# TritonDataCenter/registrar

Hardware: AMD Instinct MI355X
Metric: ephemeral registrations/sec (higher is better)
Workload: dtype n/a; 1 GPU; model=registrar re-register cycle, 1k ephemeral znodes/proc, global_batch=1000, parallelism=1 registrar procs (1/GPU), shared synthetic ZK ensemble (1 server) on rank 0, znodes_per_proc=1000, step=cleanup(1k unlink) + mkdirp + 1k ephemeral create + 1k-node heartbeat

## Files before the change

registrar_amd/csrc/bindings.cpp:

```cpp
#include <pybind11/pybind11.h>
#include <pybind11/stl.h>

#include "ensemble.hpp"
#include "gpu.hpp"
#include "health.hpp"
#include "json.hpp"
#include "log.hpp"
#include "orchestrator.hpp"
#include "registrar.hpp"
#include "zkclient.hpp"

namespace py = pybind11;
using namespace registrar;

namespace {

LogLevel level_from(const std::string& name) {
  LogLevel l = LogLevel::Warn;
  log_level_from_name(name, &l);
  return l;
}

Logger make_logger(const std::string& name, const std::string& level) {
  Logger log(name);
  log.set_level(level_from(level));
  return log;
}

py::dict stat_to_dict(const zk::Stat& st) {
  py::dict d;
  d["czxid"] = st.czxid;
  d["mzxid"] = st.mzxid;
  d["ctime"] = st.ctime;
  d["mtime"] = st.mtime;
  d["version"] = st.version;
  d["cversion"] = st.cversion;
  d["ephemeralOwner"] = st.ephemeral_owner;
  d["dataLength"] = st.data_length;
  d["numChildren"] = st.num_children;
  d["pzxid"] = st.pzxid;
  return d;
}

py::dict session_event_to_dict(const zk::SessionEvent& ev) {
  py::dict d;
  d["type"] = zk::session_event_name(ev.type);
  d["session_id"] = ev.session_id;
  d["attempt"] = ev.attempt;
  d["delay_ms"] = ev.delay_ms;
  return d;
}

py::dict orch_event_to_dict(const OrchEvent& ev) {
  py::dict d;
  d["type"] = orch_event_name(ev.type);
  d["detail"] = ev.detail;
  d["znodes"] = ev.znodes;
  d["rtt_us"] = ev.rtt_us;
  return d;
}
// ... 280 lines not shown
               rc = c.multi(mops, &per_op);
             }
             return py::make_tuple(rc, per_op);
           },
           py::arg("ops"))
      .def("heartbeat",
           [](zk::ZkClient& c, const std::vector<std::string>& nodes, const py::dict& retry) {
             zk::RetryPolicy rp = retry_from_dict(retry);
             int64_t rtt = 0;
             int rc;
             {
               py::gil_scoped_release rel;
               rc = c.heartbeat(nodes, rp, &rtt);
             }
             return py::make_tuple(rc, rtt);
           },
           py::arg("nodes"), py::arg("retry") = py::dict());

  m.def("domain_to_path", &domain_to_path);
  m.def("self_hostname", &self_hostname);
  m.def("self_address", &self_address, py::arg("admin_ip") = "");
  m.def("build_host_record",
        [](const std::string& registration_json) {
          return build_host_record(parse_registration(Json::parse(registration_json))).dump();
        });
  m.def("build_service_record",
        [](const std::string& registration_json) {
          return build_service_record(parse_registration(Json::parse(registration_json))).dump();
        });
  m.def("build_node_list",
        [](const std::string& registration_json) {
          return build_node_list(parse_registration(Json::parse(registration_json)));
        });
  py::class_<PreparedRegistration>(m, "PreparedRegistration")
      .def(py::init([](const std::string& registration_json) {
             return std::make_unique<PreparedRegistration>(
                 prepare_registration(parse_registration(Json::parse(registration_json))));
           }),
           py::arg("registration_json"))
      .def_property_readonly("path", [](const PreparedRegistration& p) { return p.path; })
      .def_property_readonly("nodes", [](const PreparedRegistration& p) { return p.nodes; })
      .def_property_readonly("host_payload",
                             [](const PreparedRegistration& p) { return py::bytes(p.host_payload); })
      .def("register_",
           [](PreparedRegistration& prep, zk::ZkClient& c, const std::string& log_level) {
             Logger log = make_logger("registrar", log_level);
             RegisterResult res;
             {
               py::gil_scoped_release rel;
               res = register_prepared(c, prep, log);
             }
             return py::make_tuple(res.rc, res.error, res.znodes());
           },
           py::arg("client"), py::arg("log_level") = "warn")
      .def("heartbeat",
           [](PreparedRegistration& prep, zk::ZkClient& c, const py::dict& retry) {
             zk::RetryPolicy rp = retry_from_dict(retry);
             int64_t rtt = 0;
             int rc;
             {
               py::gil_scoped_release rel;
               rc = heartbeat_prepared(c, prep, rp, &rtt);
             }
             return py::make_tuple(rc, rtt);
           },
           py::arg("client"), py::arg("retry") = py::dict());

  m.def("register_node",
        [](zk::ZkClient& c, const std::string& registration_json, const std::string& log_level) {
          RegistrationConfig cfg = parse_registration(Json::parse(registration_json));
          Logger log = make_logger("registrar", log_level);
          RegisterResult res;
          {
            py::gil_scoped_release rel;
            res = register_node(c, cfg, log);
          }
          return py::make_tuple(res.rc, res.error, res.znodes());
        },
        py::arg("client"), py::arg("registration_json"), py::arg("log_level") = "warn");
  m.def("unregister_node",
        [](zk::ZkClient& c, const std::vector<std::string>& znodes, const std::string& log_level) {
          Logger log = make_logger("registrar", log_level);
          py::gil_scoped_release rel;
          return unregister_node(c, znodes, log);
        },
        py::arg("client"), py::arg("znodes"), py::arg("log_level") = "warn");

  m.def("exec_with_timeout",
        [](const std::string& command, int64_t timeout_ms) {
          ExecResult res;
          {
            py::gil_scoped_release rel;
            res = exec_with_timeout(command, timeout_ms);
          }
          py::dict d;
// ... 100 lines not shown
```

registrar_amd/csrc/ensemble.cpp:

```cpp
#include "ensemble.hpp"

#include "node_store.hpp"

#include <arpa/inet.h>
#include <fcntl.h>
#include <netinet/in.h>
#include <netinet/tcp.h>
#include <sys/socket.h>
#include <unistd.h>

#include <algorithm>
#include <array>
#include <cstdio>
#include <future>

namespace registrar {
namespace zk {

using namespace detail;

namespace {

void set_nonblock(int fd) {
  int fl = fcntl(fd, F_GETFL, 0);
  fcntl(fd, F_SETFL, fl | O_NONBLOCK);
}

void set_nodelay(int fd) {
  int one = 1;
  setsockopt(fd, IPPROTO_TCP, TCP_NODELAY, &one, sizeof(one));
}

inline void spin_pause() {
#if defined(__x86_64__) || defined(__i386__)
  __builtin_ia32_pause();
// ... 409 lines not shown
        maybe_elect_leader_locked();
      }
      set_nodelay(fd);
      auto conn = std::make_shared<Conn>();
      conn->id = next_conn_id.fetch_add(1);
      conn->fd = fd;
      conn->server_idx = server_idx;
      conn->io_idx = next_io.fetch_add(1) % loops.size();
      uint64_t cid = conn->id;
      size_t io_idx = conn->io_idx;
      {
        std::lock_guard<std::mutex> g(conns_mu);
        conns[cid] = conn;
      }
      loops[io_idx]->add_fd(fd, EPOLLIN, [this, cid](uint32_t ev) { on_conn_event(cid, ev); });
    }
  }

  ConnPtr lookup(uint64_t cid) {
    std::lock_guard<std::mutex> g(conns_mu);
    auto it = conns.find(cid);
    return it == conns.end() ? nullptr : it->second;
  }

  void on_conn_event(uint64_t cid, uint32_t ev) {
    ConnPtr c = lookup(cid);
    if (!c) return;
    if (c->dead.load() || (ev & (EPOLLHUP | EPOLLERR))) {
      close_conn(c.get());
      return;
    }
    if (ev & EPOLLIN) {
      bool eof = false;
      while (true) {
        size_t room = 0;
        char* dst = c->inbuf.tail(65536, &room);
        ssize_t n = read(c->fd, dst, room);
        if (n > 0) {
          c->inbuf.commit(static_cast<size_t>(n));
        } else if (n == 0) {
          eof = true;
          break;
        } else {
          if (errno == EAGAIN || errno == EWOULDBLOCK) break;
          if (errno == EINTR) continue;
          eof = true;
          break;
        }
      }
      c->drain_mono_ms = now_ms();
      c->drain_wall_ms = wall_ms();
      c->last_parent = PathRef{std::string_view(), 0};
      {
        std::lock_guard<std::mutex> og(c->out_mu);
        c->draining = true;
      }
      if (!process_frames(c.get())) return;
      flush_out(c.get(), true);
      if (c->dead.load()) return;
      if (eof) {
        close_conn(c.get());
        return;
      }
      return;
    }
    if (ev & EPOLLOUT) flush_out(c.get());
  }

  bool process_frames(Conn* c) {
    struct CarryScope {
      Conn* c;
      Carry carry;
      explicit CarryScope(Conn* cc) : c(cc) { c->carry = &carry; }
      ~CarryScope() {
        carry.release();
        c->carry = nullptr;
      }
    } scope(c);
    while (!c->dead.load()) {
      size_t avail = c->inbuf.size();
      if (avail < 4) break;
      const unsigned char* p = reinterpret_cast<const unsigned char*>(c->inbuf.ptr());
      uint32_t len = (static_cast<uint32_t>(p[0]) << 24) | (static_cast<uint32_t>(p[1]) << 16) |
                     (static_cast<uint32_t>(p[2]) << 8) | static_cast<uint32_t>(p[3]);
      if (len > 4 * 1024 * 1024) {
        close_conn(c);
        return false;
      }
      if (avail < 4 + len) break;
      const char* body = c->inbuf.ptr() + 4;
      c->inbuf.consume(4 + len);
// ... 1440 lines not shown
```

registrar_amd/csrc/hotpath_main.cpp:

```cpp
#include <dirent.h>
#include <signal.h>
#include <sys/syscall.h>
#include <unistd.h>

#include <atomic>
#include <chrono>
#include <cstdio>
#include <cstdlib>
#include <cstring>
#include <new>
#include <set>
#include <string>
#include <vector>

#include "ensemble.hpp"
#include "registrar.hpp"
#include "zkclient.hpp"

#ifdef HOTPATH_PROF
#if !defined(__x86_64__)
#error "hotpath-prof reads x86-64 registers from the signal context"
#endif
#include <cxxabi.h>
#include <dlfcn.h>
#include <sys/time.h>
#include <ucontext.h>

#include <algorithm>
#include <map>
#endif

using namespace registrar;


namespace {
struct AllocSlot {
  std::atomic<long> tid{0};
  std::atomic<uint64_t> count{0};
  std::atomic<uint64_t> bytes{0};
};
constexpr int kMaxSlots = 256;
AllocSlot g_slots[kMaxSlots];
std::atomic<int> g_next_slot{0};
thread_local AllocSlot* t_slot = nullptr;

inline void count_alloc(size_t n) {
  AllocSlot* s = t_slot;
  if (!s) {
    int i = g_next_slot.fetch_add(1);
    if (i >= kMaxSlots) return;
// ... 222 lines not shown
  }
  return buf;
}

void prof_report() {
  size_t n = g_nsamples;
  fprintf(stderr,
          "\nhotpath-prof: %zu samples on ens-io, %zu ticks on other threads (ITIMER_PROF asked for 1 ms; the kernel "
          "delivers at its own tick rate)\n",
          n, static_cast<size_t>(g_other_thread));
  if (!n) return;
  std::map<std::string, size_t> self, chains;
  for (size_t i = 0; i < n; i++) {
    const ProfSample& s = g_samples[i];
    self[symbol_of(s.pc[0], false)]++;
    std::string c = symbol_of(s.pc[0], false);
    for (int d = 1; d < 4; d++) c += " <- " + symbol_of(s.pc[d], true);
    chains[c]++;
  }
  auto top = [&](const std::map<std::string, size_t>& m, size_t k, const char* title) {
    std::vector<std::pair<size_t, std::string>> v;
    for (auto& kv : m) v.push_back({kv.second, kv.first});
    std::sort(v.begin(), v.end(), [](auto& a, auto& b) { return a.first > b.first; });
    fprintf(stderr, "--- %s ---\n", title);
    for (size_t i = 0; i < v.size() && i < k; i++)
      fprintf(stderr, "%6.2f%% %6zu  %s\n", 100.0 * v[i].first / n, v[i].first, v[i].second.c_str());
  };
  top(self, 40, "self time per symbol");
  top(chains, 25, "most common 4-deep chains (leaf <- callers)");
}
}
#endif

int main(int argc, char** argv) {
  signal(SIGPIPE, SIG_IGN);
  int n = argc > 1 ? atoi(argv[1]) : 1000;
  int steps = argc > 2 ? atoi(argv[2]) : 200;
  int warmup = argc > 3 ? atoi(argv[3]) : 20;
  if (n < 1 || steps < 1 || warmup < 0) {
    fprintf(stderr, "usage: hotpath [N znodes >= 1] [K steps >= 1] [warmup >= 0]\n");
    return 2;
  }

  Logger log("hotpath");
  log.set_level(LogLevel::Warn);
  long caller_tid = syscall(SYS_gettid);
  name_thread(caller_tid, "caller");

  zk::EnsembleConfig ecfg;
  ecfg.ports = {0};
  ecfg.io_threads = 1;
  ecfg.max_session_timeout_ms = 60000;
  zk::Ensemble ens(ecfg);
  std::set<long> before = list_tids();
  ens.start();
  std::vector<long> ens_tids = new_tids(before);
  if (ens_tids.size() != 1) {
    fprintf(stderr, "hotpath: expected 1 ensemble IO thread, found %zu\n", ens_tids.size());
    return 1;
  }
  long ens_tid = ens_tids[0];
  name_thread(ens_tid, "ens-io");

  zk::ZkClientConfig ccfg;
  ccfg.servers.push_back({"127.0.0.1", ens.ports()[0]});
  ccfg.session_timeout_ms = 40000;
// ... 15 lines not shown
  reg.admin_ip = "127.0.0.1";
  reg.hostname = "bench-r0";
  reg.settle_ms = 0;
  for (int i = 0; i < n - 1; i++) {
    char buf[64];
    snprintf(buf, sizeof(buf), "a%04d.rank0.bench.mi355x", i);
    reg.aliases.push_back(buf);
  }
  PreparedRegistration prep = prepare_registration(reg);
  zk::RetryPolicy retry;

  auto step = [&](Sample* ens_mid) -> bool {
    RegisterResult res = register_prepared(client, prep, log);
    if (res.rc != zk::kZOk) {
      fprintf(stderr, "hotpath: register failed: %s\n", res.error.c_str());
      return false;
    }
    if (ens_mid) *ens_mid = sample_allocs(ens_tid);
    int64_t rtt = 0;
    int rc = heartbeat_prepared(client, prep, retry, &rtt);
    if (rc != zk::kZOk) {
      fprintf(stderr, "hotpath: heartbeat failed: %s\n", zk::error_name(rc));
      return false;
    }
    return true;
  };

  for (int i = 0; i < warmup; i++)
    if (!step(nullptr)) return 1;

#ifdef HOTPATH_PROF
  if (!prof_arm(ens_tid)) return 1;
#endif

  const long tids[3] = {ens_tid, cli_tid, caller_tid};
  const char* names[3] = {"ens-io", "zk-loop", "caller"};
  Sample s0[3], s1[3];
  uint64_t ens_reg_allocs = 0, ens_hb_allocs = 0;
  auto c0 = ens.counters();
  for (int t = 0; t < 3; t++) s0[t] = sample(tids[t]);
  double t0 = now_s();
  for (int i = 0; i < steps; i++) {
    Sample a = sample_allocs(ens_tid), mid;
    if (!step(&mid)) return 1;
    Sample b = sample_allocs(ens_tid);
    ens_reg_allocs += mid.allocs - a.allocs;
    ens_hb_allocs += b.allocs - mid.allocs;
  }
  double wall = now_s() - t0;
  for (int t = 0; t < 3; t++) s1[t] = sample(tids[t]);
  auto c1 = ens.counters();
  double locks_step = static_cast<double>(c1["tree_locks"] - c0["tree_locks"]) / steps;
  double locks_register = locks_step - static_cast<double>(c1["exists"] - c0["exists"]) / steps;
#ifdef HOTPATH_PROF
  prof_disarm();
#endif

  int del_rounds = steps < 5 ? steps : 5;
  uint64_t ens_del_allocs = 0;
  for (int i = 0; i < del_rounds; i++) {
    Sample a = sample_allocs(ens_tid);
    std::vector<int> rcs = client.delete_many(prep.nodes);
    Sample b = sample_allocs(ens_tid);
    for (int rc : rcs)
      if (rc != zk::kZOk) {
        fprintf(stderr, "hotpath: delete failed: %s\n", zk::error_name(rc));
        return 1;
      }
    ens_del_allocs += b.allocs - a.allocs;
    if (!step(nullptr)) return 1;
  }

  auto counters = ens.counters();
  client.close();
  ens.stop();

  double k = static_cast<double>(steps);
  fprintf(stderr, "hotpath: N=%d znodes, %d steps (+%d warmup), wall %.3f ms/step\n", n, steps, warmup,
          wall / k * 1e3);
  fprintf(stderr, "%-8s %12s %14s %14s\n", "thread", "cpu_us/step", "allocs/step", "bytes/step");
  for (int t = 0; t < 3; t++)
    fprintf(stderr, "%-8s %12.1f %14.1f %14.0f\n", names[t], (s1[t].cpu - s0[t].cpu) / k / 1e3,
            (s1[t].allocs - s0[t].allocs) / k, (s1[t].bytes - s0[t].bytes) / k);
  fprintf(stderr, "ens-io allocs by phase: register %.1f/step, heartbeat(exists) %.1f/step, delete-only %.1f/batch\n",
          ens_reg_allocs / k, ens_hb_allocs / k, ens_del_allocs / static_cast<double>(del_rounds));
  fprintf(stderr, "tree locks: %.1f/step, of which register %.1f/step\n", locks_step, locks_register);

  printf("{\"tool\": \"hotpath\", \"znodes\": %d, \"steps\": %d, \"warmup\": %d, \"wall_ms_per_step\": %.4f", n,
         steps, warmup, wall / k * 1e3);
  const char* keys[3] = {"ens_io", "zk_loop", "caller"};
  for (int t = 0; t < 3; t++)
    printf(", \"%s\": {\"cpu_us_per_step\": %.1f, \"allocs_per_step\": %.1f, \"bytes_per_step\": %.0f}", keys[t],
           (s1[t].cpu - s0[t].cpu) / k / 1e3, (s1[t].allocs - s0[t].allocs) / k, (s1[t].bytes - s0[t].bytes) / k);
  printf(", \"ens_io_allocs_register_per_step\": %.1f, \"ens_io_allocs_heartbeat_per_step\": %.1f"
         ", \"ens_io_allocs_delete_per_batch\": %.1f",
         ens_reg_allocs / k, ens_hb_allocs / k, ens_del_allocs / static_cast<double>(del_rounds));
  printf(", \"tree_locks_per_step\": %.1f, \"tree_locks_register_per_step\": %.1f", locks_step, locks_register);
  printf(", \"requests\": {\"create\": %llu, \"delete\": %llu, \"exists\": %llu}}\n",
         static_cast<unsigned long long>(counters["create"]), static_cast<unsigned long long>(counters["delete"]),
         static_cast<unsigned long long>(counters["exists"]));
#ifdef HOTPATH_PROF
  prof_report();
#endif
  return 0;
}
```

registrar_amd/csrc/stress_main.cpp:

```cpp
#include <dirent.h>
#include <execinfo.h>
#include <signal.h>
#include <sys/syscall.h>
#include <unistd.h>

#include <atomic>
#include <chrono>
#include <cstdio>
#include <cstring>
#include <thread>
#include <vector>

#include "ensemble.hpp"
#include "node_store.hpp"
#include "registrar.hpp"
#include "zkclient.hpp"

using namespace registrar;

namespace {
void dump_backtrace(int) {
  void* frames[48];
  int n = backtrace(frames, 48);
  char hdr[64];
  int len = snprintf(hdr, sizeof(hdr), "--- thread %ld backtrace ---\n", syscall(SYS_gettid));
  ssize_t r = write(2, hdr, len);
  (void)r;
  backtrace_symbols_fd(frames, n, 2);
}

void arm_watchdog(int seconds) {
  struct sigaction sa;
  memset(&sa, 0, sizeof(sa));
  sa.sa_handler = dump_backtrace;
  sigaction(SIGUSR1, &sa, nullptr);
  std::thread([seconds] {
    std::this_thread::sleep_for(std::chrono::seconds(seconds));
    fprintf(stderr, "WATCHDOG: run overshot %ds; dumping all threads\n", seconds);
    DIR* d = opendir("/proc/self/task");
    if (d) {
      while (struct dirent* e = readdir(d)) {
        if (e->d_name[0] == '.') continue;
        long tid = atol(e->d_name);
        syscall(SYS_tgkill, getpid(), tid, SIGUSR1);
        std::this_thread::sleep_for(std::chrono::milliseconds(150));
      }
      closedir(d);
    }
    std::this_thread::sleep_for(std::chrono::seconds(1));
    _exit(42);
  }).detach();
}
bool crossed_phase(int seconds, const Logger& log) {
  zk::EnsembleConfig ecfg;
  ecfg.ports = {0};
  ecfg.io_threads = 2;
  ecfg.tick_ms = 50;
  ecfg.log_level = LogLevel::Error;
  zk::Ensemble ens(ecfg);
  ens.start();
  int port = ens.ports()[0];
  auto make_client = [&] {
    zk::ZkClientConfig ccfg;
    ccfg.servers.push_back({"127.0.0.1", port});
    ccfg.session_timeout_ms = 30000;
    ccfg.log_level = LogLevel::Fatal;
    auto c = std::make_unique<zk::ZkClient>(std::move(ccfg), log);
    c->start();
    return c;
  };
  std::unique_ptr<zk::ZkClient> cl[2] = {make_client(), nullptr};
  if (!cl[0]->wait_connected(5000)) return false;
  cl[1] = make_client();
  if (!cl[1]->wait_connected(5000)) return false;
  auto reader = make_client();
  if (!reader->wait_connected(5000)) return false;
  const std::string parent[2] = {"/x/p0", "/x/p1"};
  if (cl[0]->mkdirp(parent[0]) != zk::kZOk || cl[0]->mkdirp(parent[1]) != zk::kZOk) return false;

  constexpr int kBatch = 96;
  auto batch_of = [&](int who) {
    std::vector<std::string> paths;
    for (int j = 0; j < kBatch; j++) {
      int under = ((j / 8) % 2 == 0) ? who : 1 - who;
      paths.push_back(parent[under] + "/s" + std::to_string(who) + "_" + std::to_string(j));
// ... 225 lines not shown
          break;
        }
        case 2: {
          for (size_t i = 0; i < 3; i++)
            if (!ens.server_up(i)) ens.restart_server(i);
          break;
        }
        default:
          ens.set_latency_ms(static_cast<int>(next() % 3));
          break;
      }
    }
    ens.set_latency_ms(0);
    for (size_t i = 0; i < 3; i++)
      if (!ens.server_up(i)) ens.restart_server(i);
  };

  for (int phase = 0; phase < 2; phase++) {
    bool contested = phase == 1;
    int secs = contested ? contested_seconds : seconds;
    if (secs <= 0) continue;
    stop.store(false);
    std::vector<std::thread> threads;
    for (int i = 0; i < nclients; i++) threads.emplace_back(client_fn, i, contested);
    std::thread chaos(chaos_fn);
    std::this_thread::sleep_for(std::chrono::seconds(secs));
    stop.store(true);
    for (auto& t : threads) t.join();
    chaos.join();
  }

  bool crossed_ok = crossed_secs <= 0 || crossed_phase(crossed_secs, log);
  bool treelock_ok = treelock_phase();

  auto deadline = std::chrono::steady_clock::now() + std::chrono::seconds(15);
  while (!ens.session_ids().empty() && std::chrono::steady_clock::now() < deadline)
    std::this_thread::sleep_for(std::chrono::milliseconds(20));
  size_t sessions_left = ens.session_ids().size();
  std::vector<std::string> violations = ens.audit();
  deadline = std::chrono::steady_clock::now() + std::chrono::seconds(2);
  while (!violations.empty() && std::chrono::steady_clock::now() < deadline) {
    std::this_thread::sleep_for(std::chrono::milliseconds(20));
    violations = ens.audit();
  }
  size_t ephemerals_left = ens.ephemeral_count();
  ens.stop();

  printf("stress: %llu cycles, %llu hard failures, %llu contested cycles\n",
         static_cast<unsigned long long>(cycles.load()), static_cast<unsigned long long>(failures.load()),
         static_cast<unsigned long long>(contested_cycles.load()));
  bool sound = true;
  if (sessions_left != 0) {
    printf("stress: %zu sessions still alive after every client closed\n", sessions_left);
    sound = false;
  }
  if (ephemerals_left != 0) {
    printf("stress: %zu ephemerals left\n", ephemerals_left);
    sound = false;
  }
  for (const auto& v : violations) {
    printf("stress: audit: %s\n", v.c_str());
    sound = false;
  }
  if (contested_seconds > 0 && contested_cycles.load() == 0) {
    printf("stress: the contested phase completed no cycle\n");
    sound = false;
  }
  bool behaved = cycles.load() > 0 && failures.load() < cycles.load() / 4 + 16;
  if (!crossed_ok) printf("stress: the crossed-parents phase failed\n");
  if (!treelock_ok) printf("stress: the tree lock phase failed\n");
  return (behaved && sound && crossed_ok && treelock_ok) ? 0 : 1;
}
```

registrar_amd/csrc/zkclient.cpp:

```cpp
#include "zkclient.hpp"

#include <arpa/inet.h>
#include <fcntl.h>
#include <netdb.h>
#include <netinet/in.h>
#include <netinet/tcp.h>
#include <sys/socket.h>
#include <unistd.h>

#include <algorithm>
#include <chrono>
#include <future>
#include <thread>
#include <unordered_set>

namespace registrar {
namespace zk {

const char* session_event_name(SessionEvent::Type t) {
  switch (t) {
    case SessionEvent::Type::Connected:
      return "connect";
    case SessionEvent::Type::Disconnected:
      return "close";
    case SessionEvent::Type::Expired:
      return "session_expired";
    case SessionEvent::Type::ConnectAttempt:
      return "attempt";
    case SessionEvent::Type::Closed:
      return "closed";
  }
  return "?";
}
// ... 269 lines not shown
  void teardown_socket() {
    if (conn_timer) {
      loop.cancel(conn_timer);
      conn_timer = 0;
    }
    if (ping_timer) {
      loop.cancel(ping_timer);
      ping_timer = 0;
    }
    if (fd >= 0) {
      loop.del_fd(fd);
      ::close(fd);
      fd = -1;
    }
    inbuf.clear();
    outbuf.clear();
    flush_scheduled = false;
  }

  void fail_all_pending(int rc) {
    std::deque<Pending> q;
    q.swap(pending);
    for (auto& p : q) {
      if (p.rcs)
        fail_batch(p, rc);
      else if (p.done)
        p.done(rc, nullptr);
    }
  }


  bool read_frames() {
    bool eof = false;
    while (true) {
      size_t room = 0;
      char* dst = inbuf.tail(65536, &room);
      ssize_t n = read(fd, dst, room);
      if (n > 0) {
        inbuf.commit(static_cast<size_t>(n));
      } else if (n == 0) {
        eof = true;
        break;
      } else {
        if (errno == EAGAIN || errno == EWOULDBLOCK) break;
        if (errno == EINTR) continue;
        eof = true;
        break;
      }
    }
    last_recv = now_ms();
    while (true) {
      size_t avail = inbuf.size();
      if (avail < 4) break;
      const unsigned char* p = reinterpret_cast<const unsigned char*>(inbuf.ptr());
      uint32_t len = (static_cast<uint32_t>(p[0]) << 24) | (static_cast<uint32_t>(p[1]) << 16) |
                     (static_cast<uint32_t>(p[2]) << 8) | static_cast<uint32_t>(p[3]);
      if (len > 64 * 1024 * 1024) {
        on_connection_lost("oversized frame");
        return false;
      }
      if (avail < 4 + len) break;
      const char* body = inbuf.ptr() + 4;
      inbuf.consume(4 + len);
      if (!handle_frame(body, len)) return false;
    }
    if (eof) {
      if (fd >= 0) on_connection_lost("eof");
      return false;
    }
    return true;
  }

  bool handle_frame(const char* body, size_t len) {
    try {
      JuteReader r(body, len);
      if (phase == Phase::Handshaking) {
        ConnectResponse resp;
        resp.deserialize(r);
        if (conn_timer) {
          loop.cancel(conn_timer);
          conn_timer = 0;
        }
        if (resp.session_id == 0 || resp.time_out_ms <= 0) {
          if (have_session) {
            log.warn("zookeeper: session expired by server", {{"session", Json(sid)}});
            teardown_socket();
            fail_all_pending(kZSessionExpired);
            data_watch_paths.clear();
            exist_watch_paths.clear();
            child_watch_paths.clear();
            phase = Phase::Stopped;
            state.store(SessionState::Expired);
            emit({SessionEvent::Type::Expired, sid, 0, 0});
          } else {
            on_connect_failed("handshake rejected");
          }
          return false;
        }
        bool reconnected = have_session;
        have_session = true;
// ... 43 lines not shown
            break;
          default:
            data_watch_paths.erase(ev.path);
            exist_watch_paths.erase(ev.path);
            break;
        }
        {
          std::lock_guard<std::mutex> g(watch_mu);
          watch_queue.push_back(ev);
        }
        if (watch_cb) watch_cb(ev);
        return true;
      }
      if (pending.empty()) {
        on_connection_lost("unexpected reply");
        return false;
      }
      if (pending.front().rcs) {
        Pending& bp = pending.front();
        int32_t want = xid_add(bp.xid, bp.next);
        if (want != hdr.xid) {
          log.error("zookeeper: xid mismatch", {{"expected", Json(static_cast<int64_t>(want))},
                                                {"got", Json(static_cast<int64_t>(hdr.xid))}});
          Pending failed = std::move(bp);
          pending.pop_front();
          fail_batch(failed, kZConnectionLoss);
          on_connection_lost("xid mismatch");
          return false;
        }
        (*bp.rcs)[bp.next++] = hdr.err;
        if (bp.next == bp.count) {
          BatchWaiter* wtr = bp.waiter;
          pending.pop_front();
          wtr->signal();
        }
        return true;
      }
      Pending p = std::move(pending.front());
      pending.pop_front();
      if (p.xid != hdr.xid) {
        log.error("zookeeper: xid mismatch", {{"expected", Json(static_cast<int64_t>(p.xid))},
                                              {"got", Json(static_cast<int64_t>(hdr.xid))}});
        if (p.done) p.done(kZConnectionLoss, nullptr);
        on_connection_lost("xid mismatch");
        return false;
      }
      if (p.done) {
        p.done(hdr.err, &r);
      }
      return true;
    } catch (const std::exception& e) {
      log.error("zookeeper: malformed frame", {{"err", Json(e.what())}});
      on_connection_lost("malformed frame");
      return false;
    }
  }


  void schedule_ping() {
    int64_t interval = std::max<int64_t>(negotiated_timeout / 3, 100);
    ping_timer = loop.schedule(interval, [this] {
      ping_timer = 0;
      if (phase != Phase::Ready) return;
      if (now_ms() - last_recv > negotiated_timeout * 2 / 3) {
        on_connection_lost("ping timeout");
        return;
// ... 15 lines not shown
    JuteWriter w(&outbuf);
    RequestHeader hdr;
    hdr.xid = xid;
    hdr.type = op;
    hdr.serialize(w);
    serialize_body(w);
    uint32_t n = static_cast<uint32_t>(outbuf.size() - start - 4);
    outbuf[start] = static_cast<char>(n >> 24);
    outbuf[start + 1] = static_cast<char>(n >> 16);
    outbuf[start + 2] = static_cast<char>(n >> 8);
    outbuf[start + 3] = static_cast<char>(n);
    Pending p;
    p.xid = xid;
    p.op = op;
    p.done = std::move(done);
    pending.push_back(std::move(p));
    schedule_flush();
  }

  template <typename SerFn>
  void submit_op(int32_t op, SerFn serialize_body, std::function<void(int, JuteReader*)> done) {
    submit(next_xid++, op, serialize_body, std::move(done));
  }

  void schedule_flush() {
    if (flush_scheduled) return;
    flush_scheduled = true;
    loop.schedule(0, [this] {
      flush_scheduled = false;
      flush(false);
    });
  }

  void flush(bool from_epollout) {
    if (fd < 0) return;
    size_t off = 0;
    while (off < outbuf.size()) {
      ssize_t n = send(fd, outbuf.data() + off, outbuf.size() - off, MSG_NOSIGNAL);
      if (n > 0) {
        off += static_cast<size_t>(n);
      } else if (n < 0 && (errno == EAGAIN || errno == EWOULDBLOCK)) {
        break;
      } else if (n < 0 && errno == EINTR) {
        continue;
      } else {
        on_connection_lost("write error");
        return;
      }
    }
    outbuf.erase(0, off);
    if (!outbuf.empty()) {
      loop.mod_fd(fd, EPOLLIN | EPOLLOUT);
    } else if (from_epollout) {
      loop.mod_fd(fd, EPOLLIN);
    }
  }
};


ZkClient::ZkClient(ZkClientConfig cfg, Logger log) : impl_(std::make_unique<Impl>(std::move(cfg), log)) {
  if (impl_->cfg.servers.empty()) throw std::runtime_error("ZkClient: options.servers empty");
}

ZkClient::~ZkClient() {
  try {
    close();
  } catch (...) {
  }
}

void ZkClient::start() {
  if (impl_->started.exchange(true)) return;
  impl_->thread = std::thread([this] {
    impl_->loop.post([this] { impl_->start_connect(); });
    impl_->loop.run();
  });
}

bool ZkClient::wait_connected(int64_t timeout_ms) {
  std::unique_lock<std::mutex> g(impl_->ev_mu);
  auto pred = [this] { return impl_->settled; };
  if (timeout_ms < 0) {
// ... 496 lines not shown
    t.ops.push_back(mo.op);
  }
  return t;
}

ZkClient::BatchTemplate ZkClient::make_exists_template(const std::vector<std::string>& paths) {
  BatchTemplate t;
  for (const auto& path : paths) {
    size_t start = t.buf.size();
    t.buf.append(4, '\0');
    t.xid_offsets.push_back(t.buf.size());
    JuteWriter w(&t.buf);
    w.write_int(0);
    w.write_int(kOpExists);
    w.write_string(path);
    w.write_bool(false);
    uint32_t n = static_cast<uint32_t>(t.buf.size() - start - 4);
    t.buf[start] = static_cast<char>(n >> 24);
    t.buf[start + 1] = static_cast<char>(n >> 16);
    t.buf[start + 2] = static_cast<char>(n >> 8);
    t.buf[start + 3] = static_cast<char>(n);
    t.ops.push_back(kOpExists);
  }
  return t;
}

std::vector<int> ZkClient::submit_template(BatchTemplate& t) {
  size_t n = t.xid_offsets.size();
  std::vector<int> rcs(n, kZConnectionLoss);
  if (n == 0) return rcs;
  Impl::BatchWaiter waiter;
  Impl::BatchWaiter* wp = &waiter;
  std::vector<int>* rp = &rcs;
  impl_->loop.post([this, &t, wp, rp, n] {
    if (impl_->phase != Impl::Phase::Ready) {
      int rc = impl_->phase == Impl::Phase::Stopped ? kZSessionExpired : kZConnectionLoss;
      for (size_t i = 0; i < n; i++) (*rp)[i] = rc;
      wp->signal();
      return;
    }
    int32_t first = impl_->next_xid;
    for (size_t i = 0; i < n; i++) {
      uint32_t u = static_cast<uint32_t>(Impl::xid_add(first, static_cast<uint32_t>(i)));
      size_t off = t.xid_offsets[i];
      t.buf[off] = static_cast<char>(u >> 24);
      t.buf[off + 1] = static_cast<char>(u >> 16);
      t.buf[off + 2] = static_cast<char>(u >> 8);
      t.buf[off + 3] = static_cast<char>(u);
    }
    impl_->next_xid = Impl::xid_add(first, static_cast<uint32_t>(n));
    Impl::Pending p;
    p.xid = first;
    p.op = t.ops[0];
    p.rcs = rp;
    p.count = static_cast<uint32_t>(n);
    p.waiter = wp;
    impl_->pending.push_back(std::move(p));
    impl_->outbuf += t.buf;
    impl_->schedule_flush();
  });
  waiter.wait();
  return rcs;
}

int ZkClient::heartbeat_template(BatchTemplate& t, const RetryPolicy& retry, int64_t* rtt_us) {
  Backoff bo;
  bo.initial_ms = retry.initial_delay_ms;
  bo.max_ms = retry.max_delay_ms;
  bo.max_attempts = retry.max_attempts;
  while (true) {
    int64_t t0 = now_us();
    std::vector<int> rcs = submit_template(t);
    int rc = kZOk;
    for (int r : rcs) {
      if (r != kZOk) {
        rc = r;
        break;
      }
    }
    if (rc == kZOk) {
      if (rtt_us) *rtt_us = now_us() - t0;
      return kZOk;
    }
    SessionState st = state();
    if (rc == kZSessionExpired || st == SessionState::Expired || st == SessionState::Closed) return rc;
    if (bo.exhausted()) return rc;
    int64_t delay = bo.next_delay();
    std::unique_lock<std::mutex> g(impl_->ev_mu);
    impl_->ev_cv.wait_for(g, std::chrono::milliseconds(delay), [this] {
      SessionState s2 = impl_->state.load();
      return impl_->closed.load() || s2 == SessionState::Expired || s2 == SessionState::Closed;
    });
    if (impl_->closed.load()) return kZConnectionLoss;
  }
// ... 38 lines not shown
```

Baseline: 4.848 million registrations/s.

## Send batch templates in place, bulk-parse batch replies, cache loggers and result lists

Batch templates are now sent directly from the caller's buffer when the client outbuf is empty, which avoids a string copy and a deferred flush hop through the event loop. Consecutive batch reply headers are parsed in a tight loop straight into the rc vector instead of going through per-frame handling. The Python binding caches the Logger per level and reuses a prebuilt Python list of registered nodes, returning a slice copy. The change also adds opt-in tracing instrumentation and a stress pipeline phase, and the fast reply parser brings some risk to correctness on malformed or interleaved frames.

```diff
diff --git a/registrar_amd/csrc/bindings.cpp b/registrar_amd/csrc/bindings.cpp
--- a/registrar_amd/csrc/bindings.cpp
+++ b/registrar_amd/csrc/bindings.cpp
@@ -26,6 +26,28 @@
   log.set_level(level_from(level));
   return log;
 }
+
+const Logger& registrar_logger(const std::string& level) {
+  static std::unique_ptr<Logger> cache[static_cast<int>(LogLevel::Fatal) / 10 + 1];
+  std::unique_ptr<Logger>& slot = cache[static_cast<int>(level_from(level)) / 10];
+  if (!slot) slot = std::make_unique<Logger>(make_logger("registrar", level));
+  return *slot;
+}
+
+struct PyPrepared {
+  PreparedRegistration prep;
+  py::object registered;
+
+  explicit PyPrepared(PreparedRegistration p) : prep(std::move(p)) {}
+
+  py::list registered_list() {
+    if (!registered) registered = py::cast(*prep.registered_nodes);
+    PyObject* src = registered.ptr();
+    PyObject* copy = PyList_GetSlice(src, 0, PyList_GET_SIZE(src));
+    if (!copy) throw py::error_already_set();
+    return py::reinterpret_steal<py::list>(copy);
+  }
+};
 
 py::dict stat_to_dict(const zk::Stat& st) {
   py::dict d;
@@ -372,35 +394,37 @@
         [](const std::string& registration_json) {
           return build_node_list(parse_registration(Json::parse(registration_json)));
         });
-  py::class_<PreparedRegistration>(m, "PreparedRegistration")
+  py::class_<PyPrepared>(m, "PreparedRegistration")
       .def(py::init([](const std::string& registration_json) {
-             return std::make_unique<PreparedRegistration>(
+             return std::make_unique<PyPrepared>(
                  prepare_registration(parse_registration(Json::parse(registration_json))));
            }),
            py::arg("registration_json"))
-      .def_property_readonly("path", [](const PreparedRegistration& p) { return p.path; })
-      .def_property_readonly("nodes", [](const PreparedRegistration& p) { return p.nodes; })
+      .def_property_readonly("path", [](const PyPrepared& p) { return p.prep.path; })
+      .def_property_readonly("nodes", [](const PyPrepared& p) { return p.prep.nodes; })
       .def_property_readonly("host_payload",
-                             [](const PreparedRegistration& p) { return py::bytes(p.host_payload); })
+                             [](const PyPrepared& p) { return py::bytes(p.prep.host_payload); })
       .def("register_",
-           [](PreparedRegistration& prep, zk::ZkClient& c, const std::string& log_level) {
-             Logger log = make_logger("registrar", log_level);
+           [](PyPrepared& p, zk::ZkClient& c, const std::string& log_level) -> py::tuple {
+             const Logger& log = registrar_logger(log_level);
              RegisterResult res;
              {
                py::gil_scoped_release rel;
-               res = register_prepared(c, prep, log);
-             }
+               res = register_prepared(c, p.prep, log);
+             }
+             if (res.rc == zk::kZOk && res.nodes == p.prep.registered_nodes)
+               return py::make_tuple(res.rc, res.error, p.registered_list());
              return py::make_tuple(res.rc, res.error, res.znodes());
            },
            py::arg("client"), py::arg("log_level") = "warn")
       .def("heartbeat",
-           [](PreparedRegistration& prep, zk::ZkClient& c, const py::dict& retry) {
+           [](PyPrepared& p, zk::ZkClient& c, const py::dict& retry) {
              zk::RetryPolicy rp = retry_from_dict(retry);
              int64_t rtt = 0;
              int rc;
              {
                py::gil_scoped_release rel;
-               rc = heartbeat_prepared(c, prep, rp, &rtt);
+               rc = heartbeat_prepared(c, p.prep, rp, &rtt);
              }
              return py::make_tuple(rc, rtt);
            },
diff --git a/registrar_amd/csrc/ensemble.cpp b/registrar_amd/csrc/ensemble.cpp
--- a/registrar_amd/csrc/ensemble.cpp
+++ b/registrar_amd/csrc/ensemble.cpp
@@ -1,6 +1,7 @@
 #include "ensemble.hpp"
 
 #include "node_store.hpp"
+#include "trace.hpp"
 
 #include <arpa/inet.h>
 #include <fcntl.h>
@@ -476,12 +477,14 @@
     }
     if (ev & EPOLLIN) {
       bool eof = false;
+      [[maybe_unused]] size_t got = 0;
       while (true) {
         size_t room = 0;
         char* dst = c->inbuf.tail(65536, &room);
         ssize_t n = read(c->fd, dst, room);
         if (n > 0) {
           c->inbuf.commit(static_cast<size_t>(n));
+          got += static_cast<size_t>(n);
         } else if (n == 0) {
           eof = true;
           break;
@@ -492,6 +495,7 @@
           break;
         }
       }
+      HP_TRACE(kSrvRead, got);
       c->drain_mono_ms = now_ms();
       c->drain_wall_ms = wall_ms();
       c->last_parent = PathRef{std::string_view(), 0};
@@ -500,7 +504,9 @@
         c->draining = true;
       }
       if (!process_frames(c.get())) return;
+      HP_TRACE(kSrvHandled, c->stage.size());
       flush_out(c.get(), true);
+      HP_TRACE(kSrvFlushed, 0);
       if (c->dead.load()) return;
       if (eof) {
         close_conn(c.get());
diff --git a/registrar_amd/csrc/hotpath_main.cpp b/registrar_amd/csrc/hotpath_main.cpp
--- a/registrar_amd/csrc/hotpath_main.cpp
+++ b/registrar_amd/csrc/hotpath_main.cpp
@@ -16,6 +16,14 @@
 #include "ensemble.hpp"
 #include "registrar.hpp"
 #include "zkclient.hpp"
+
+#ifdef HOTPATH_TRACE
+#include <time.h>
+
+#include <algorithm>
+
+#include "trace.hpp"
+#endif
 
 #ifdef HOTPATH_PROF
 #if !defined(__x86_64__)
@@ -304,6 +312,178 @@
 }
 #endif
 
+#ifdef HOTPATH_TRACE
+
+namespace {
+struct TraceRec {
+  uint64_t ns;
+  uint32_t point;
+  uint32_t arg;
+};
+constexpr size_t kTraceCap = 1 << 21;
+TraceRec* g_trace = nullptr;
+std::atomic<size_t> g_trace_n{0};
+std::atomic<bool> g_trace_on{false};
+
+const char* kPointNames[registrar::trace::kPoints] = {
+    "step",           "caller posts",   "caller awake",  "client lambda",   "client send start", "client send end",
+    "client read",    "client parsed",  "client signal", "server read",     "server handled",    "server flushed"};
+}
+
+namespace registrar::trace {
+void mark(Point p, uint32_t arg) {
+  if (!g_trace_on.load(std::memory_order_relaxed)) return;
+  struct timespec ts;
+  clock_gettime(CLOCK_MONOTONIC, &ts);
+  size_t i = g_trace_n.fetch_add(1, std::memory_order_relaxed);
+  if (i >= kTraceCap) return;
+  g_trace[i] = TraceRec{static_cast<uint64_t>(ts.tv_sec) * 1000000000ull + static_cast<uint64_t>(ts.tv_nsec), p, arg};
+}
+}
+
+namespace {
+constexpr int kLegs = 9;
+const char* kLegNames[kLegs] = {"caller posts -> client lambda runs",
+                                "lambda -> send starts",
+                                "client send",
+                                "send done -> server has read everything",
+                                "server read everything -> last frames handled",
+                                "last frames handled -> last flush done",
+                                "last flush done -> client has read all replies",
+                                "client parses replies, signals",
+                                "signal -> caller awake"};
+
+struct BatchSum {
+  double leg[kLegs] = {0};
+  double total = 0, handle_sum = 0, flush_sum = 0;
+  double srv_reads = 0, srv_flushes = 0, cli_reads = 0, bytes_in = 0, bytes_out = 0;
+  size_t n = 0;
+};
+
+bool sum_batch(const TraceRec* r, size_t a, size_t b, BatchSum* out) {
+  using namespace registrar::trace;
+  uint64_t post = r[a].ns, lambda = 0, ss = 0, se = 0, read_all = 0, handled = 0, flushed = 0, cli_read = 0, sig = 0,
+           awake = 0, last_srv_read = 0;
+  double handle_sum = 0, flush_sum = 0, srv_reads = 0, srv_flushes = 0, cli_reads = 0, in = 0, outb = 0;
+  for (size_t i = a + 1; i < b; i++) {
+    const TraceRec& x = r[i];
+    switch (x.point) {
+      case kCliLambda:
+        if (!lambda) lambda = x.ns;
+        break;
+      case kCliSendStart:
+        if (lambda && !ss && x.arg) ss = x.ns;
+        break;
+      case kCliSendEnd:
+        if (ss && x.arg) se = x.ns;
+        break;
+      case kSrvRead:
+        last_srv_read = x.ns;
+        if (x.arg) {
+          read_all = x.ns;
+          srv_reads += 1;
+          in += x.arg;
+        }
+        break;
+      case kSrvHandled:
+        if (last_srv_read) handle_sum += (x.ns - last_srv_read) / 1e3;
+        handled = x.ns;
+        outb += x.arg;
+        break;
+      case kSrvFlushed:
+        if (handled) flush_sum += (x.ns - handled) / 1e3;
+        flushed = x.ns;
+        last_srv_read = x.ns;
+        srv_flushes += 1;
+        break;
+      case kCliRead:
+        if (x.arg) {
+          cli_read = x.ns;
+          cli_reads += 1;
+        }
+        break;
+      case kCliSignal:
+        sig = x.ns;
+        break;
+      case kCallerAwake:
+        awake = x.ns;
+        break;
+      default:
+        break;
+    }
+  }
+  if (!lambda || !ss || !se || !read_all || !handled || !flushed || !cli_read || !sig || !awake) return false;
+  const uint64_t chain[kLegs + 1] = {post, lambda, ss, se, read_all, handled, flushed, cli_read, sig, awake};
+  for (int l = 0; l < kLegs; l++)
+    out->leg[l] += (static_cast<double>(chain[l + 1]) - static_cast<double>(chain[l])) / 1e3;
+  out->total += (awake - post) / 1e3;
+  out->handle_sum += handle_sum;
+  out->flush_sum += flush_sum;
+  out->srv_reads += srv_reads;
+  out->srv_flushes += srv_flushes;
+  out->cli_reads += cli_reads;
+  out->bytes_in += in;
+  out->bytes_out += outb;
+  out->n++;
+  return true;
+}
+
+void trace_report(int steps) {
+  using namespace registrar::trace;
+  size_t n = std::min(g_trace_n.load(), kTraceCap);
+  std::stable_sort(g_trace, g_trace + n, [](const TraceRec& x, const TraceRec& y) { return x.ns < y.ns; });
+  std::vector<size_t> step_at;
+  for (size_t i = 0; i < n; i++)
+    if (g_trace[i].point == kStep) step_at.push_back(i);
+  step_at.push_back(n);
+  BatchSum sums[2];
+  size_t skipped = 0;
+  for (size_t s = 0; s + 1 < step_at.size(); s++) {
+    std::vector<size_t> posts;
+    for (size_t i = step_at[s]; i < step_at[s + 1]; i++)
+      if (g_trace[i].point == kCallerPost) posts.push_back(i);
+    posts.push_back(step_at[s + 1]);
+    for (size_t k = 0; k + 1 < posts.size() && k < 2; k++)
+      if (!sum_batch(g_trace, posts[k], posts[k + 1], &sums[k])) skipped++;
+    bool late = static_cast<int>(s) == steps - 3 || static_cast<int>(s) == steps - 2;
+    if (late || (steps < 3 && s == 0)) {
+      fprintf(stderr, "\n--- timeline of step %zu (us from the step's first post) ---\n", s);
+      uint64_t t0 = 0;
+      for (size_t i = step_at[s]; i < step_at[s + 1]; i++) {
+        const TraceRec& x = g_trace[i];
+        if (x.point == kStep) continue;
+        if (!t0) t0 = x.ns;
+        fprintf(stderr, "%9.1f  %-18s %u\n", (x.ns - t0) / 1e3, kPointNames[x.point], x.arg);
+      }
+    }
+  }
+  const char* kinds[2] = {"register batch", "heartbeat"};
+  fprintf(stderr, "\n--- legs per batch, mean over %zu timed steps (us) ---\n", sums[0].n);
+  fprintf(stderr, "%-48s %16s %16s\n", "leg", kinds[0], kinds[1]);
+  auto mean = [](double v, const BatchSum& b) { return b.n ? v / b.n : 0.0; };
+  for (int l = 0; l < kLegs; l++)
+    fprintf(stderr, "%-48s %16.1f %16.1f\n", kLegNames[l], mean(sums[0].leg[l], sums[0]), mean(sums[1].leg[l], sums[1]));
+  fprintf(stderr, "%-48s %16.1f %16.1f\n", "total", mean(sums[0].total, sums[0]), mean(sums[1].total, sums[1]));
+  fprintf(stderr, "%-48s %16.1f %16.1f\n", "server handling, summed over drains",
+          mean(sums[0].handle_sum, sums[0]), mean(sums[1].handle_sum, sums[1]));
+  fprintf(stderr, "%-48s %16.1f %16.1f\n", "server flushes, summed", mean(sums[0].flush_sum, sums[0]),
+          mean(sums[1].flush_sum, sums[1]));
+  fprintf(stderr, "%-48s %16.2f %16.2f\n", "server reads with data", mean(sums[0].srv_reads, sums[0]),
+          mean(sums[1].srv_reads, sums[1]));
+  fprintf(stderr, "%-48s %16.2f %16.2f\n", "server flushes", mean(sums[0].srv_flushes, sums[0]),
+          mean(sums[1].srv_flushes, sums[1]));
+  fprintf(stderr, "%-48s %16.2f %16.2f\n", "client reads with data", mean(sums[0].cli_reads, sums[0]),
+          mean(sums[1].cli_reads, sums[1]));
+  fprintf(stderr, "%-48s %16.0f %16.0f\n", "bytes in / batch", mean(sums[0].bytes_in, sums[0]),
+          mean(sums[1].bytes_in, sums[1]));
+  fprintf(stderr, "%-48s %16.0f %16.0f\n", "bytes staged / batch", mean(sums[0].bytes_out, sums[0]),
+          mean(sums[1].bytes_out, sums[1]));
+  if (skipped) fprintf(stderr, "(%zu batches lacked a mark and were left out of the means)\n", skipped);
+  if (g_trace_n.load() > kTraceCap) fprintf(stderr, "(trace array full: later marks were dropped)\n");
+}
+}
+#endif
+
 int main(int argc, char** argv) {
   signal(SIGPIPE, SIG_IGN);
   int n = argc > 1 ? atoi(argv[1]) : 1000;
@@ -385,6 +565,11 @@
 #ifdef HOTPATH_PROF
   if (!prof_arm(ens_tid)) return 1;
 #endif
+#ifdef HOTPATH_TRACE
+  g_trace = static_cast<TraceRec*>(calloc(kTraceCap, sizeof(TraceRec)));
+  if (!g_trace) return 1;
+  g_trace_on.store(true);
+#endif
 
   const long tids[3] = {ens_tid, cli_tid, caller_tid};
   const char* names[3] = {"ens-io", "zk-loop", "caller"};
@@ -394,6 +579,9 @@
   for (int t = 0; t < 3; t++) s0[t] = sample(tids[t]);
   double t0 = now_s();
   for (int i = 0; i < steps; i++) {
+#ifdef HOTPATH_TRACE
+    registrar::trace::mark(registrar::trace::kStep, static_cast<uint32_t>(i));
+#endif
     Sample a = sample_allocs(ens_tid), mid;
     if (!step(&mid)) return 1;
     Sample b = sample_allocs(ens_tid);
@@ -407,6 +595,9 @@
   double locks_register = locks_step - static_cast<double>(c1["exists"] - c0["exists"]) / steps;
 #ifdef HOTPATH_PROF
   prof_disarm();
+#endif
+#ifdef HOTPATH_TRACE
+  g_trace_on.store(false);
 #endif
 
   int del_rounds = steps < 5 ? steps : 5;
@@ -455,5 +646,8 @@
 #ifdef HOTPATH_PROF
   prof_report();
 #endif
+#ifdef HOTPATH_TRACE
+  trace_report(steps);
+#endif
   return 0;
 }
diff --git a/registrar_amd/csrc/stress_main.cpp b/registrar_amd/csrc/stress_main.cpp
--- a/registrar_amd/csrc/stress_main.cpp
+++ b/registrar_amd/csrc/stress_main.cpp
@@ -51,6 +51,118 @@
     _exit(42);
   }).detach();
 }
+bool pipeline_phase(int rounds, const Logger& log) {
+  zk::EnsembleConfig ecfg;
+  ecfg.ports = {0};
+  ecfg.io_threads = 2;
+  ecfg.tick_ms = 50;
+  ecfg.log_level = LogLevel::Error;
+  zk::Ensemble ens(ecfg);
+  ens.start();
+  int port = ens.ports()[0];
+  auto make_client = [&] {
+    zk::ZkClientConfig ccfg;
+    ccfg.servers.push_back({"127.0.0.1", port});
+    ccfg.session_timeout_ms = 30000;
+    ccfg.log_level = LogLevel::Fatal;
+    auto c = std::make_unique<zk::ZkClient>(std::move(ccfg), log);
+    c->start();
+    return c;
+  };
+  std::unique_ptr<zk::ZkClient> cl[2] = {make_client(), nullptr};
+  if (!cl[0]->wait_connected(5000)) return false;
+  cl[1] = make_client();
+  if (!cl[1]->wait_connected(5000)) return false;
+  auto watcher = make_client();
+  if (!watcher->wait_connected(5000)) return false;
+  const std::string parent[2] = {"/pipe/p0", "/pipe/p1"};
+  if (cl[0]->mkdirp(parent[0]) != zk::kZOk || cl[0]->mkdirp(parent[1]) != zk::kZOk) return false;
+
+  constexpr int kCreates = 3000, kDeletes = 4500;
+  std::atomic<bool> stop{false};
+  std::atomic<int> bad{0};
+  std::atomic<uint64_t> events{0};
+  auto worker = [&](int who) {
+    const std::string& under = parent[1 - who];
+    auto name = [&](int i) {
+      char buf[96];
+      snprintf(buf, sizeof(buf), "%s/s%d-%05d-padding-to-make-the-path-long-enough", under.c_str(), who, i);
+      return std::string(buf);
+    };
+    std::vector<zk::ZkClient::MixedOp> creates, deletes;
+    std::vector<std::string> created;
+    for (int i = 0; i < kCreates; i++) {
+      zk::ZkClient::MixedOp op;
+      op.op = zk::kOpCreate;
+      op.path = name(i);
+      op.data = std::string(40, 'd');
+      op.flags = zk::kEphemeral;
+      created.push_back(op.path);
+      creates.push_back(std::move(op));
+    }
+    for (int j = 0; j < kDeletes; j++) {
+      zk::ZkClient::MixedOp op;
+      op.op = zk::kOpDelete;
+      op.path = j % 3 == 2 ? name(100000 + j) : name(j - j / 3);
+      deletes.push_back(std::move(op));
+    }
+    auto create_tpl = zk::ZkClient::make_template(creates);
+    auto delete_tpl = zk::ZkClient::make_template(deletes);
+    auto exists_tpl = zk::ZkClient::make_exists_template(created);
+    char peer_first[96];
+    snprintf(peer_first, sizeof(peer_first), "%s/s%d-%05d-padding-to-make-the-path-long-enough", parent[who].c_str(),
+             1 - who, 0);
+    auto arm = [&] {
+      int rc = cl[who]->exists(peer_first, nullptr, true);
+      if (rc != zk::kZOk && rc != zk::kZNoNode) bad.fetch_add(1);
+      events.fetch_add(cl[who]->poll_watches().size());
+    };
+    for (int r = 0; r < rounds && !bad.load(); r++) {
+      arm();
+      std::vector<int> rcs = cl[who]->submit_template(create_tpl);
+      for (int i = 0; i < kCreates; i++)
+        if (rcs[i] != zk::kZOk) bad.fetch_add(1);
+      arm();
+      rcs = cl[who]->submit_template(exists_tpl);
+      for (int i = 0; i < kCreates; i++)
+        if (rcs[i] != zk::kZOk) bad.fetch_add(1);
+      arm();
+      rcs = cl[who]->submit_template(delete_tpl);
+      for (int j = 0; j < kDeletes; j++)
+        if (rcs[j] != (j % 3 == 2 ? zk::kZNoNode : zk::kZOk)) bad.fetch_add(1);
+      rcs = cl[who]->submit_template(exists_tpl);
+      for (int i = 0; i < kCreates; i++)
+        if (rcs[i] != zk::kZNoNode) bad.fetch_add(1);
+    }
+  };
+  std::thread watch_thread([&] {
+    std::vector<std::string> kids;
+    while (!stop.load()) {
+      for (int p = 0; p < 2; p++)
+        if (watcher->get_children(parent[p], &kids, true) != zk::kZOk) bad.fetch_add(1);
+      events.fetch_add(watcher->poll_watches().size());
+    }
+  });
+  std::thread w0(worker, 0), w1(worker, 1);
+  w0.join();
+  w1.join();
+  stop.store(true);
+  watch_thread.join();
+  std::vector<std::string> kids;
+  bool empty = true;
+  for (int p = 0; p < 2; p++)
+    if (cl[0]->get_children(parent[p], &kids) != zk::kZOk || !kids.empty()) empty = false;
+  std::vector<std::string> violations = ens.audit();
+  size_t eph = ens.ephemeral_count();
+  for (auto& c : cl) c->close();
+  watcher->close();
+  ens.stop();
+  printf("stress: pipeline phase: %d rounds x 2 sessions, %llu watch events, %d wrong return codes\n", rounds,
+         static_cast<unsigned long long>(events.load()), bad.load());
+  for (const auto& v : violations) printf("stress: pipeline audit: %s\n", v.c_str());
+  return bad.load() == 0 && empty && violations.empty() && eph == 0 && events.load() > 0;
+}
+
 bool crossed_phase(int seconds, const Logger& log) {
   zk::EnsembleConfig ecfg;
   ecfg.ports = {0};
@@ -342,6 +454,7 @@
 
   bool crossed_ok = crossed_secs <= 0 || crossed_phase(crossed_secs, log);
   bool treelock_ok = treelock_phase();
+  bool pipeline_ok = crossed_secs <= 0 || pipeline_phase(12, log);
 
   auto deadline = std::chrono::steady_clock::now() + std::chrono::seconds(15);
   while (!ens.session_ids().empty() && std::chrono::steady_clock::now() < deadline)
@@ -379,5 +492,6 @@
   bool behaved = cycles.load() > 0 && failures.load() < cycles.load() / 4 + 16;
   if (!crossed_ok) printf("stress: the crossed-parents phase failed\n");
   if (!treelock_ok) printf("stress: the tree lock phase failed\n");
-  return (behaved && sound && crossed_ok && treelock_ok) ? 0 : 1;
-}
+  if (!pipeline_ok) printf("stress: the pipeline phase failed\n");
+  return (behaved && sound && crossed_ok && treelock_ok && pipeline_ok) ? 0 : 1;
+}
diff --git a/registrar_amd/csrc/trace.hpp b/registrar_amd/csrc/trace.hpp
--- /dev/null
+++ b/registrar_amd/csrc/trace.hpp
@@ -0,0 +1,28 @@
+#pragma once
+
+#ifdef HOTPATH_TRACE
+#include <cstdint>
+
+namespace registrar::trace {
+enum Point : uint32_t {
+  kStep = 0,
+  kCallerPost,
+  kCallerAwake,
+  kCliLambda,
+  kCliSendStart,
+  kCliSendEnd,
+  kCliRead,
+  kCliParsed,
+  kCliSignal,
+  kSrvRead,
+  kSrvHandled,
+  kSrvFlushed,
+  kPoints
+};
+void mark(Point p, uint32_t arg);
+}
+
+#define HP_TRACE(point, arg) ::registrar::trace::mark(::registrar::trace::point, static_cast<uint32_t>(arg))
+#else
+#define HP_TRACE(point, arg) ((void)0)
+#endif
diff --git a/registrar_amd/csrc/zkclient.cpp b/registrar_amd/csrc/zkclient.cpp
--- a/registrar_amd/csrc/zkclient.cpp
+++ b/registrar_amd/csrc/zkclient.cpp
@@ -1,4 +1,6 @@
 #include "zkclient.hpp"
+
+#include "trace.hpp"
 
 #include <arpa/inet.h>
 #include <fcntl.h>
@@ -334,12 +336,14 @@
 
   bool read_frames() {
     bool eof = false;
+    [[maybe_unused]] size_t got = 0;
     while (true) {
       size_t room = 0;
       char* dst = inbuf.tail(65536, &room);
       ssize_t n = read(fd, dst, room);
       if (n > 0) {
         inbuf.commit(static_cast<size_t>(n));
+        got += static_cast<size_t>(n);
       } else if (n == 0) {
         eof = true;
         break;
@@ -350,8 +354,10 @@
         break;
       }
     }
+    HP_TRACE(kCliRead, got);
     last_recv = now_ms();
     while (true) {
+      if (!batch_replies()) return false;
       size_t avail = inbuf.size();
       if (avail < 4) break;
       const unsigned char* p = reinterpret_cast<const unsigned char*>(inbuf.ptr());
@@ -366,8 +372,41 @@
       inbuf.consume(4 + len);
       if (!handle_frame(body, len)) return false;
     }
+    HP_TRACE(kCliParsed, 0);
     if (eof) {
       if (fd >= 0) on_connection_lost("eof");
+      return false;
+    }
+    return true;
+  }
+
+  bool batch_replies() {
+    if (phase != Phase::Ready || pending.empty() || !pending.front().rcs) return true;
+    Pending& bp = pending.front();
+    if (bp.next + 1 >= bp.count) return true;
+    try {
+      const char* p = inbuf.ptr();
+      size_t avail = inbuf.size(), used = 0;
+      int* rcs = bp.rcs->data();
+      uint32_t next = bp.next;
+      const uint32_t last = bp.count - 1;
+      int64_t zxid = last_zxid;
+      while (next < last && avail - used >= 4 + ReplyHeader::kWireSize) {
+        JuteReader r(p + used, 4 + ReplyHeader::kWireSize);
+        uint32_t len = static_cast<uint32_t>(r.read_int());
+        if (len < ReplyHeader::kWireSize || len > avail - used - 4) break;
+        if (r.read_int() != xid_add(bp.xid, next)) break;
+        int64_t z = r.read_long();
+        if (z > 0) zxid = z;
+        rcs[next++] = r.read_int();
+        used += 4 + len;
+      }
+      bp.next = next;
+      last_zxid = zxid;
+      inbuf.consume(used);
+    } catch (const std::exception& e) {
+      log.error("zookeeper: malformed frame", {{"err", Json(e.what())}});
+      on_connection_lost("malformed frame");
       return false;
     }
     return true;
@@ -477,6 +516,7 @@
         if (bp.next == bp.count) {
           BatchWaiter* wtr = bp.waiter;
           pending.pop_front();
+          HP_TRACE(kCliSignal, 0);
           wtr->signal();
         }
         return true;
@@ -558,9 +598,33 @@
     });
   }
 
+  void send_in_place(const std::string& buf) {
+    size_t off = 0;
+    HP_TRACE(kCliSendStart, buf.size());
+    while (off < buf.size()) {
+      ssize_t n = send(fd, buf.data() + off, buf.size() - off, MSG_NOSIGNAL);
+      if (n > 0) {
+        off += static_cast<size_t>(n);
+      } else if (n < 0 && (errno == EAGAIN || errno == EWOULDBLOCK)) {
+        break;
+      } else if (n < 0 && errno == EINTR) {
+        continue;
+      } else {
+        on_connection_lost("write error");
+        return;
+      }
+    }
+    HP_TRACE(kCliSendEnd, off);
+    if (off < buf.size()) {
+      outbuf.assign(buf, off, buf.size() - off);
+      loop.mod_fd(fd, EPOLLIN | EPOLLOUT);
+    }
+  }
+
   void flush(bool from_epollout) {
     if (fd < 0) return;
     size_t off = 0;
+    HP_TRACE(kCliSendStart, outbuf.size());
     while (off < outbuf.size()) {
       ssize_t n = send(fd, outbuf.data() + off, outbuf.size() - off, MSG_NOSIGNAL);
       if (n > 0) {
@@ -574,6 +638,7 @@
         return;
       }
     }
+    HP_TRACE(kCliSendEnd, off);
     outbuf.erase(0, off);
     if (!outbuf.empty()) {
       loop.mod_fd(fd, EPOLLIN | EPOLLOUT);
@@ -1136,7 +1201,9 @@
   Impl::BatchWaiter waiter;
   Impl::BatchWaiter* wp = &waiter;
   std::vector<int>* rp = &rcs;
+  HP_TRACE(kCallerPost, n);
   impl_->loop.post([this, &t, wp, rp, n] {
+    HP_TRACE(kCliLambda, 0);
     if (impl_->phase != Impl::Phase::Ready) {
       int rc = impl_->phase == Impl::Phase::Stopped ? kZSessionExpired : kZConnectionLoss;
       for (size_t i = 0; i < n; i++) (*rp)[i] = rc;
@@ -1160,10 +1227,15 @@
     p.count = static_cast<uint32_t>(n);
     p.waiter = wp;
     impl_->pending.push_back(std::move(p));
+    if (impl_->outbuf.empty() && impl_->fd >= 0) {
+      impl_->send_in_place(t.buf);
+      return;
+    }
     impl_->outbuf += t.buf;
     impl_->schedule_flush();
   });
   waiter.wait();
+  HP_TRACE(kCallerAwake, 0);
   return rcs;
 }
 
```

New measurement: 5.618 million registrations/s, median of 3. 15.9% higher.
